# bit-bots/SoccerDiffusion

Hardware: AMD Instinct MI355X
Metric: denoised joint-trajectories/s (50-step DDIM, H=100, J=20) (higher is better)
Workload: dtype f32 (operands split into fp16 hi+lo, 3 fp16 MFMAs per product at every site, fp32 accumulate: 22-bit operands; single noise prediction vs the fp64 oracle 8e-7 on these weights and 2e-6 on weights stressed to |logit| ~ 60 (tests/test_gpu_denoiser.py::test_mode3_noise_prediction_single_step); valid fo; 1 GPU; BASELINE.json configs[2]: 50-step DDIM sampling, B=4096 parallel rollouts per GPU, transformer denoiser d=256 L=4 heads=4, horizon T=100, J=20, memory M=11 (10 context tokens + step token); one step = one full rollout; the timed region issues the rollout's launches eagerly.  Kernel selection: sampler mode 3 (--sampler-mode); batch_per_gpu=4096, ddim_steps=50, horizon=100, joints=20, hidden_dim=256, decoder_layers=4, parallelism=dp1 (independent rollouts, no collective)

## Files before the change

include/soccerdiffusion_hip.h:

```cpp
#ifndef SOCCERDIFFUSION_HIP_H
#define SOCCERDIFFUSION_HIP_H

#include <stddef.h>
#include <stdint.h>

#ifdef __cplusplus
extern "C" {
#endif

#define SD_ABI_VERSION 1

#define SD_E_BADARG (-1)
#define SD_E_BADDIM (-2)
#define SD_E_TOOBIG (-3)
#define SD_E_UNSUPPORTED (-4)

typedef struct sd_layer_weights {
    const float *sa_in_w;
    const float *sa_in_b;
    const float *sa_out_w;
    const float *sa_out_b;
    const float *ca_in_w;
    const float *ca_in_b;
    const float *ca_out_w;
// ... 38 lines not shown
int sd_abi_version(void);
const char *sd_last_error(void);

size_t sd_workspace_floats(int B, int T, int M, int d, int L, int n_steps);

#define SD_ROUTE_CHAINS_F32 0
#define SD_ROUTE_CHAINS_F16 1
#define SD_ROUTE_FUSED 2
#define SD_ROUTE_FUSED_FOLD 3
#define SD_ROUTE_FUSED_FOLD_F16 4
#define SD_ROUTE_TRAJ_TUNED 5
#define SD_ROUTE_TRAJ_TUNED_2P 6
#define SD_ROUTE_TRAJ_TUNED_WIDE 7
#define SD_ROUTE_TRAJ_GENERIC 8
int sd_sampler_route(int d, int heads, int T, int Mc, int J, int L, int B, int max_mode);
int sd_sampler_mode(int d, int heads, int T, int Mc, int J);

int sd_step_token(const void *steps, int steps_is_i64, const float *freq, const float *token,
                  float *out, long out_row_stride, int B, int d, void *stream);

int sd_denoiser_forward(const sd_denoiser_weights *w, const float *x, const float *memory,
                        float *eps_out, float *workspace, int B, int T, int M, void *stream);

int sd_encoder_forward(const sd_encoder_weights *w, const float *x, float *out,
                       float *workspace, int B, int S, void *stream);

int sd_game_state_embed(const int64_t *idx, const float *table, float *out, long out_row_stride,
                        int B, int d, int n_states, void *stream);

int sd_ddim_add_noise(const float *x0, const float *noise, const int64_t *t, const float *acp,
// ... 305 lines not shown
```

soccerdiffusion_amd/_lib.py:

```python

from __future__ import annotations

import ctypes as C
import os

import torch

_PKG = os.path.dirname(os.path.abspath(__file__))
LIB_PATH = os.environ.get("SD_HIP_LIB") or os.path.join(_PKG, "lib", "libsoccerdiffusion_hip.so")

c_float_p = C.POINTER(C.c_float)


class LayerWeights(C.Structure):

    FIELDS = (
        "sa_in_w", "sa_in_b", "sa_out_w", "sa_out_b",
        "ca_in_w", "ca_in_b", "ca_out_w", "ca_out_b",
        "lin1_w", "lin1_b", "lin2_w", "lin2_b",
        "n1_w", "n1_b", "n2_w", "n2_b", "n3_w", "n3_b",
    )
    _fields_ = [(n, C.c_void_p) for n in FIELDS]


# ... 189 lines not shown
    "sd_session_commit_carry_at": (C.c_int, [C.c_void_p] * 7 + [C.c_int] * 7 + [C.c_void_p] * 3),
    "sd_session_reset_carry": (C.c_int, [C.POINTER(RingReset), C.c_int, C.c_void_p, C.c_void_p, C.c_int64, C.c_void_p, C.c_int, C.c_void_p]),
    "sd_profile_enable": (C.c_int, [C.c_int]),
    "sd_profile_collect": (C.c_int, [C.POINTER(C.c_double), C.POINTER(C.c_long), C.c_int]),
}

ROUTES = ("CHAINS_F32", "CHAINS_F16", "FUSED", "FUSED_FOLD", "FUSED_FOLD_F16", "TRAJ_TUNED", "TRAJ_TUNED_2P", "TRAJ_TUNED_WIDE", "TRAJ_GENERIC")


def sampler_route(d: int, heads: int, T: int, Mc: int, J: int, L: int, B: int, max_mode: int = -1) -> str:
    rc = load().sd_sampler_route(d, heads, T, Mc, J, L, B, max_mode)
    check(min(rc, 0), "sd_sampler_route")
    return ROUTES[rc]


KERNEL_CLASSES = ("panel_gemm_kernel", "attention_kernel", "patch_embed_kernel", "fc_out_kernel", "decoder_layer_kernel", "decoder_head_kernel",
                  "traj_step_kernel")

_lib = None


def load() -> C.CDLL:
    global _lib
    if _lib is not None:
        return _lib
    if not os.path.exists(LIB_PATH):
        raise RuntimeError(
            f"{LIB_PATH} is missing: build it with `python -m soccerdiffusion_amd.build` "
            "(hipcc, gfx950).  soccerdiffusion_amd has no CPU fallback."
        )
# ... 17 lines not shown
```

soccerdiffusion_amd/csrc/sd_kernels.hip:

```cpp

#include <hip/hip_runtime.h>
#include <stdint.h>
#include <math.h>
#include <algorithm>
#include <cstdlib>
#include <cstring>

#include "../../include/soccerdiffusion_hip.h"

#include "sd_common.h"
#include "sd_panel.h"

static thread_local const char *g_last_error = "ok";
int fail(int code, const char *msg) {
    g_last_error = msg;
    return code;
}

const unsigned *g_dropout_epoch = nullptr;
extern "C" int sd_set_dropout_epoch(const uint32_t *device_word) {
    g_dropout_epoch = device_word;
    return 0;
}

// ... 2619 lines not shown
        return fail(SD_E_BADDIM, "hidden_dim must be one of 64, 128, 256, 512");
    if (w->p <= 0 || S / w->p <= 0 || S / w->p > w->S_max)
        return fail(SD_E_TOOBIG, "sd_encoder_forward: sequence exceeds positional table");
    hipStream_t st = (hipStream_t)stream;
    const int d = w->d, n = S / w->p, R = B * n;
    Scratch s = carve(workspace, R, 1, d, 1, 0);
    int rc = patch_embed(x, w->emb_w, w->emb_b, w->pe, s.h, B, S, w->C, w->p, d, st);
    if (rc) return rc;
    if ((rc = encoder_stack(w->layers, w->L, s, B, n, d, w->heads, st))) return rc;
    SD_LAUNCH(copy_rows_kernel, dim3(grid_for((long)R * d)), dim3(256), 0, st, s.h, (long)d, out, (long)d,
                       (long)R, d);
    SD_CHECK_LAUNCH("copy_rows_kernel");
    return 0;
}

extern "C" int sd_sampler_mode(int d, int heads, int T, int Mc, int J) { return sampler_plan(d, heads, T, Mc, J, 1, 1, 3).mode(); }

extern "C" int sd_sampler_route(int d, int heads, int T, int Mc, int J, int L, int B, int max_mode) {
    if (max_mode < -1 || max_mode > 4) return fail(SD_E_BADARG, "sd_sampler_route: max_mode must be -1, 0, 1, 2, 3 or 4");
    return sampler_plan(d, heads, T, Mc, J, L, B, max_mode < 0 ? 3 : max_mode).route;
}

extern "C" int sd_ddim_sample(const sd_denoiser_weights *w, const float *ctx, const float *step_tokens,
                              const float *coef, float *x, float *trace, float *workspace, int B, int T, int Mc,
                              int n_steps, void *stream) {
    return sd_ddim_sample_eps(w, ctx, step_tokens, coef, x, trace, nullptr, workspace, B, T, Mc, n_steps, nullptr, -1, stream);
}

extern "C" int sd_ddim_sample_ex(const sd_denoiser_weights *w, const float *ctx, const float *step_tokens,
                                 const float *coef, float *x, float *trace, float *workspace, int B, int T, int Mc,
                                 int n_steps, int32_t *status, int max_mode, void *stream) {
    return sd_ddim_sample_eps(w, ctx, step_tokens, coef, x, trace, nullptr, workspace, B, T, Mc, n_steps, status, max_mode, stream);
}


// ... 38 lines not shown
    const long n = (long)B * T * J;
    SD_LAUNCH(ddim_pin_kernel, dim3(grid_for(n)), dim3(256), 0, st, x, pin, ck, cn, n, T, J);
    SD_CHECK_LAUNCH("ddim_pin_kernel");
    return 0;
}

static int traj_rollout(const TrajCall &c, const float *ctx, const float *step_tokens, const float *coef, float *x, float *trace, float *eps_trace,
                        int32_t *status, const PinArgs *pin = nullptr) {
    const long n = (long)c.B * c.T * c.w->J;
    int rc;
    if (status && (rc = zero_async(status, sizeof(int32_t), c.st))) return rc;
    if ((rc = c.prepare_weights())) return rc;
    if ((rc = c.prepare_ctx(ctx))) return rc;
    if ((rc = c.prepare_steps(step_tokens, false))) return rc;
    if (pin && (rc = ddim_pin(x, *pin, coef[0], coef[1], c.B, c.T, c.w->J, c.st))) return rc;
    for (int i = 0; i < c.n_tok; ++i) {
        float *eps_i = eps_trace ? eps_trace + (size_t)i * n : nullptr;
        if ((rc = c.step(x, eps_i, i, coef + 4 * i, false, status, pin))) return rc;
        if (trace && (rc = trace_copy(x, trace, i, n, c.st))) return rc;
    }
    return status ? finite_check(x, n, status, c.st) : 0;
}

static int panel_rollout(const sd_denoiser_weights *w, const Scratch &s, const SamplerPlan &plan, const float *ctx, const float *step_tokens,
                         const float *coef, float *x, float *trace, float *eps_trace, int B, int T, int Mc, int n_steps, int32_t *status, hipStream_t st,
                         const PinArgs *pin = nullptr) {
    const int d = w->d, R = B * T, L = w->L;
    int rc;
    const int Mk = Mc + 1;
    const size_t kvstride = (size_t)B * Mk * 2 * d, kvsstride = (size_t)n_steps * 2 * d;
// ... 67 lines not shown
}

static int ddim_sample_any(const sd_denoiser_weights *w, const float *ctx, const float *step_tokens, const float *coef, float *x, float *trace,
                           float *eps_trace, float *workspace, int B, int T, int Mc, int n_steps, int32_t *status, int max_mode, void *stream,
                           const PinArgs *pin) {
    int rc = check_denoiser(w);
    if (rc) return rc;
    if (!step_tokens || !coef || !x || !workspace || B <= 0 || T <= 0 || Mc < 0 || n_steps <= 0 || (Mc > 0 && !ctx))
        return fail(SD_E_BADARG, "sd_ddim_sample: null pointer or empty shape");
    if (max_mode < -1 || max_mode > 4) return fail(SD_E_BADARG, "sd_ddim_sample_ex: max_mode must be -1, 0, 1, 2, 3 or 4");
    if (max_mode < 0) max_mode = 3;
    if (max_mode == 4 && !status) return fail(SD_E_BADARG, "sd_ddim_sample_ex: max_mode 4 needs a status word (SD_STATUS_SHARP_LOGITS)");
    if (T > w->T_max) return fail(SD_E_TOOBIG, "sd_ddim_sample: horizon exceeds positional table");
    hipStream_t st = (hipStream_t)stream;
    const Scratch s = carve(workspace, (long)B * T, (long)B * (Mc + 1), w->d, w->L, n_steps, B);
    const SamplerPlan plan = sampler_plan(w->d, w->heads, T, Mc, w->J, w->L, B, max_mode);
    if (plan.traj()) return traj_rollout(TrajCall{plan, w, s, B, T, Mc, n_steps, st}, ctx, step_tokens, coef, x, trace, eps_trace, status, pin);
    return panel_rollout(w, s, plan, ctx, step_tokens, coef, x, trace, eps_trace, B, T, Mc, n_steps, status, st, pin);
}

extern "C" int sd_ddim_sample_eps(const sd_denoiser_weights *w, const float *ctx, const float *step_tokens,
                                  const float *coef, float *x, float *trace, float *eps_trace, float *workspace, int B, int T, int Mc,
                                  int n_steps, int32_t *status, int max_mode, void *stream) {
    return ddim_sample_any(w, ctx, step_tokens, coef, x, trace, eps_trace, workspace, B, T, Mc, n_steps, status, max_mode, stream, nullptr);
}

extern "C" int sd_ddim_sample_pin(const sd_denoiser_weights *w, const float *ctx, const float *step_tokens, const float *coef, float *x,
                                  float *trace, float *eps_trace, float *workspace, int B, int T, int Mc, int n_steps, int32_t *status,
                                  int max_mode, const float *pin_x0, const float *pin_noise, const int32_t *pin_rows, void *stream) {
    if (!pin_x0 || !pin_noise || !pin_rows) return fail(SD_E_BADARG, "sd_ddim_sample_pin: pin_x0, pin_noise and pin_rows must be given");
    if (pin_noise == x) return fail(SD_E_BADARG, "sd_ddim_sample_pin: pin_noise must not alias x (x is overwritten by the first step)");
    const PinArgs pin{pin_x0, pin_noise, pin_rows};
    return ddim_sample_any(w, ctx, step_tokens, coef, x, trace, eps_trace, workspace, B, T, Mc, n_steps, status, max_mode == 4 ? 3 : max_mode,
                           stream, &pin);
}

static int sampler_eval_args(const sd_denoiser_weights *w, float *workspace, int B, int T, int Mc, int n_tok, int max_mode, const char *who,
                             Scratch *s, SamplerPlan *plan) {
    int rc = check_denoiser(w);
    if (rc) return rc;
    if (!workspace || B <= 0 || T <= 0 || Mc < 0 || (n_tok != 1 && n_tok != B)) return fail(SD_E_BADARG, who);
    if (max_mode < -1 || max_mode > 4) return fail(SD_E_BADARG, who);
    if (T > w->T_max) return fail(SD_E_TOOBIG, who);
    *s = carve(workspace, (long)B * T, (long)B * (Mc + 1), w->d, w->L, n_tok, B);
    *plan = sampler_plan(w->d, w->heads, T, Mc, w->J, w->L, B, max_mode < 0 ? 3 : max_mode);
    return plan->traj() ? 0 : SD_E_UNSUPPORTED;
}

extern "C" int sd_sampler_prepare(const sd_denoiser_weights *w, const float *ctx, float *workspace, int B, int T, int Mc, int n_tok,
                                  int what, int max_mode, void *stream) {
    Scratch s;
    SamplerPlan plan;
    int rc = sampler_eval_args(w, workspace, B, T, Mc, n_tok, max_mode, "sd_sampler_prepare: bad argument", &s, &plan);
    if (rc) return rc;
    if ((what & ~(SD_PREPARE_WEIGHTS | SD_PREPARE_CONTEXT)) || (Mc > 0 && (what & SD_PREPARE_CONTEXT) && !ctx))
        return fail(SD_E_BADARG, "sd_sampler_prepare: bad argument");
    const TrajCall c{plan, w, s, B, T, Mc, n_tok, (hipStream_t)stream};
    if ((what & SD_PREPARE_WEIGHTS) && (rc = c.prepare_weights())) return rc;
    if ((what & SD_PREPARE_CONTEXT) && (rc = c.prepare_ctx(ctx))) return rc;
    return 0;
// ... 142 lines not shown
```

soccerdiffusion_amd/csrc/sd_sampler_plan.h:

```cpp
#ifndef SD_SAMPLER_PLAN_H
#define SD_SAMPLER_PLAN_H
#include <stdlib.h>
#include <string.h>

#include "../../include/soccerdiffusion_hip.h"

bool traj_ok(int d, int heads, int T, int Mk, int J, int L);
bool trajg_ok(int d, int heads, int T, int Mk, int J, int L);

inline bool fused_layer_ok(int d, int heads, int T, int Mk) {
    if (heads != 4 || d < 128) return false;
    const int n_traj = (63 + T - 1) / T + 1;
    return (long)n_traj * Mk <= 64;
}

struct SamplerSwitches {
    bool traj, f16, trajg;
    int max_rows;
};
inline const SamplerSwitches &sampler_switches() {
    static const SamplerSwitches sw = [] {
        const auto is = [](const char *name, const char *value) {
            const char *e = getenv(name);
            return e && strcmp(e, value) == 0;
        };
        const char *mr = getenv("SD_TRAJ_MAXROWS");
        return SamplerSwitches{!is("SD_SAMPLER_TRAJ", "0"), !is("SD_SAMPLER_GEMM", "f32"), !is("SD_SAMPLER_TRAJG", "0"), mr ? atoi(mr) : 64};
    }();
    return sw;
}

struct SamplerPlan {
    int route;
    int key_tiles;
    bool precise;
    bool kv_fp32;
    bool fused, fold, f16, chain16;
    bool traj() const { return route >= SD_ROUTE_TRAJ_TUNED; }
    int mode() const { return traj() ? 3 : route == SD_ROUTE_FUSED_FOLD_F16 ? 2 : route == SD_ROUTE_FUSED_FOLD ? 1 : 0; }
};

inline SamplerPlan panel_plan(int d, int heads, int T, int Mk, int J, int B, int cap) {
    const SamplerSwitches &sw = sampler_switches();
    const bool layer_ok = fused_layer_ok(d, heads, T, Mk);
    SamplerPlan p{};
    p.kv_fp32 = cap < 2;
    p.fused = layer_ok && (long)B * Mk * 2 * d < (1L << 30);
    p.fold = cap >= 1 && p.fused && heads == 4 && d >= 128 && Mk <= 16 && T >= 64;
    p.f16 = cap >= 2 && p.fold && sw.f16 && d == 256 && J % 4 == 0;
    p.chain16 = cap >= 2 && !p.fold && !layer_ok && sw.f16 && (d == 128 || d == 256 || d == 512) && J % 4 == 0;
    p.route = p.f16 ? SD_ROUTE_FUSED_FOLD_F16 : p.fold ? SD_ROUTE_FUSED_FOLD : p.fused ? SD_ROUTE_FUSED : p.chain16 ? SD_ROUTE_CHAINS_F16 : SD_ROUTE_CHAINS_F32;
    return p;
}

inline SamplerPlan sampler_plan(int d, int heads, int T, int Mc, int J, int L, int B, int max_mode) {
    const SamplerSwitches &sw = sampler_switches();
    const int Mk = Mc + 1;
    if (max_mode >= 3 && sw.traj && sw.f16) {
        if ((long)B * Mk * 2 * d < (1L << 30) && Mk <= sw.max_rows && traj_ok(d, heads, T, Mk, J, L)) {
            SamplerPlan p{};
            p.key_tiles = (Mk + 15) / 16;
            p.precise = max_mode == 3 || p.key_tiles > 1;
            p.route = p.key_tiles > 1 ? SD_ROUTE_TRAJ_TUNED_WIDE : p.precise ? SD_ROUTE_TRAJ_TUNED : SD_ROUTE_TRAJ_TUNED_2P;
            return p;
        }
        if (sw.trajg && trajg_ok(d, heads, T, Mk, J, L)) {
            SamplerPlan p{};
            p.route = SD_ROUTE_TRAJ_GENERIC;
            return p;
        }
    }
    return panel_plan(d, heads, T, Mk, J, B, max_mode < 2 ? max_mode : 2);
}
#endif
```

soccerdiffusion_amd/csrc/sd_traj.h:

```cpp
#pragma once
#include "sd_common.h"
#include "sd_mfma16.h"
#include "soccerdiffusion_hip.h"
#include <type_traits>

namespace tj {

constexpr int D = 256, HD = 64, NH = 4, TMAX = 100;
constexpr int NTHREADS = 512;
constexpr int MAX_L = 8;
constexpr float ACT = 8.0f;
constexpr float PSC = 1024.0f;
constexpr float XSC = 1.0f;
constexpr int XROW = 1024, X1ROW = 512, QROW = 256, VROW = 288, PROW = 512;
constexpr int LDS_X = 0;
constexpr int LDS_SQ = LDS_X + TMAX * X1ROW;
constexpr int LDS_SO = LDS_SQ + TMAX * QROW;
constexpr int LDS_Q = LDS_X + TMAX * XROW;
constexpr int LDS_K = LDS_Q + TMAX * QROW;
constexpr int LDS_P = LDS_Q;
constexpr int LDS_STAT = LDS_K + TMAX * VROW;
constexpr int LDS_BYTES = LDS_STAT + TMAX * 8 * 8;
static_assert(LDS_SO + TMAX * QROW <= LDS_Q, "Q and O fit the freed half of the panel");
static_assert(LDS_BYTES <= 163840 && LDS_P + TMAX * PROW <= LDS_STAT, "LDS budget");
// ... 6 lines not shown
constexpr int TJ_NSTAMP = 96, TJ_STAMP_WGS = 512;
__device__ unsigned long long *g_tj_stamps;
#define TJ_STAMP(i)                                                                                                            \
    do {                                                                                                                       \
        if (blockIdx.x < TJ_STAMP_WGS && (threadIdx.x & 63) == 0)                                                              \
            g_tj_stamps[((long)blockIdx.x * 8 + (threadIdx.x >> 6)) * TJ_NSTAMP + (i)] = __builtin_amdgcn_s_memtime();        \
    } while (0)
template <int SITE>
__device__ __forceinline__ void tj_sync() {
    const unsigned long long t0 = __builtin_amdgcn_s_memtime();
    __syncthreads();
    const unsigned long long t1 = __builtin_amdgcn_s_memtime();
    if (blockIdx.x < TJ_STAMP_WGS && (threadIdx.x & 63) == 0) g_tj_stamps[((long)blockIdx.x * 8 + (threadIdx.x >> 6)) * TJ_NSTAMP + 64 + SITE] += t1 - t0;
}
#define TJ_SYNC(site) tj_sync<site>()
#else
#define TJ_STAMP(i) do {} while (0)
#define TJ_SYNC(site) __syncthreads()
#endif

#ifndef TJ_DROP_ALO
#define TJ_DROP_ALO 0
#endif
#ifndef TJ_DROP_BLO
#define TJ_DROP_BLO 0
#endif
enum Site { S_QKV = 1, S_SCORES = 2, S_PV = 4, S_OUT = 8, S_XSC = 16, S_XPV = 32, S_W1 = 64, S_W2 = 128, S_EMB = 256, S_FC = 512 };
template <int SITE = 0>
__device__ __forceinline__ void mma3(f32x4 &c, f16x8 ah, f16x8 al, f16x8 bh, f16x8 bl) {
    if constexpr ((TJ_DROP_ALO | TJ_DROP_BLO) & SITE) {
        if constexpr (!(TJ_DROP_ALO & SITE)) c = mfma16(al, bh, c);
        if constexpr (!(TJ_DROP_BLO & SITE)) c = mfma16(ah, bl, c);
        c = mfma16(ah, bh, c);
// ... 171 lines not shown
    const float *b_emb, *pe;
    const float *n1_w, *n1_b;
    const f16 *w_out;
    const float *b_out;
    const float *sc_io;
    float c0, c1, c2, c3;
    float scale_log2e;
    int T, B, J, L, Mk, update_x;
    int nkt;
    const int *step_map;
    int step_per_traj;
    int *status;
    LayerW layer[MAX_L];
};

template <int NTT, bool PRECISE>
struct TJ {
static constexpr int LAST0 = 16 * (NTT - 1);
static constexpr int NH0 = (NTT + 1) / 2;
static constexpr int NKP = (NTT + 1) / 2;


static __device__ __forceinline__ void ctx_init(Ctx &c, char *smem, int T) {
    c.smem = smem;
    c.lane = threadIdx.x & 63;
    c.w = __builtin_amdgcn_readfirstlane(threadIdx.x >> 6);
    c.g = c.lane >> 4;
    c.t = c.lane & 15;
    c.T = T;
    c.ok6 = LAST0 + c.t < T;
    c.tok6 = c.ok6 ? LAST0 + c.t : T - 1;
#pragma unroll
    for (int m2 = 0; m2 < 4; ++m2) {
        const unsigned in_row = (unsigned)(((c.g ^ (c.t & 3)) << 4) + ((m2 ^ (c.t >> 2)) << 6));
        const unsigned in_row6 = (unsigned)(((c.g ^ (c.tok6 & 3)) << 4) + ((m2 ^ ((c.tok6 >> 2) & 3)) << 6));
        c.xa[m2] = (unsigned)(c.t * XROW) + in_row;
        c.xa6[m2] = (unsigned)(c.tok6 * XROW) + in_row6;
    }
}

static __device__ __forceinline__ Ctx ctx_local(const Ctx &c) {
    Ctx d;
    d.smem = c.smem;
    d.lane = c.lane;
    asm volatile("" : "+v"(d.lane));
    d.w = c.w;
    d.g = d.lane >> 4;
    d.t = d.lane & 15;
    d.T = c.T;
    d.ok6 = LAST0 + d.t < d.T;
    d.tok6 = d.ok6 ? LAST0 + d.t : d.T - 1;
#pragma unroll
    for (int m2 = 0; m2 < 4; ++m2) {
// ... 782 lines not shown
            for (int pl = 0; pl < 2; ++pl) svv[n][pl] = vstep[(pl * 4 + c.g) * D + 16 * (2 * c.w + n) + c.t];
        }
        __builtin_amdgcn_sched_barrier(0);
        auto scores = [&](auto odd_c) __attribute__((always_inline)) {
            constexpr bool OD = decltype(odd_c)::value;
            constexpr int N1 = OD ? NTT - NH0 : NH0, T1 = OD ? NH0 : 0;
            constexpr int N1D = N1 > 0 ? N1 : 1;
            f16x8 xb[3][2];
            ring_pipe<8 * N1, 3>(
                [&](int s) __attribute__((always_inline)) {
                    xb[s % 3][0] = lds16(X + x_at(c, T1 + s % N1D, 0, s / N1D));
                    xb[s % 3][1] = lds16(X + x_at(c, T1 + s % N1D, 1, s / N1D));
                },
                [&](int s) __attribute__((always_inline)) { mma3<S_XSC>(S[s % N1D], gfr[s / N1D][0], gfr[s / N1D][1], xb[s % 3][0], xb[s % 3][1]); });
        };
        if (odd) scores(std::true_type{});
        else scores(std::false_type{});
#pragma unroll
        for (int n = 0; n < 2; ++n)
#pragma unroll
            for (int pl = 0; pl < 2; ++pl) av[n][2][pl] = f16x8{svv[n][pl], 0, 0, 0, 0, 0, 0, 0};
        const float c_g = 1.0f / (ACT * sc4);
        const StepScale ss = step_scale(sc5, sc6, sc7);
        f32x4 cg4 = {c_g, c_g, c_g, c_g};
#pragma unroll
        for (int r = 0; r < 4; ++r)
            if (4 * c.g + r == Mc) {
                cbv[r] = cs;
                cg4[r] = ss.c_gs;
            }
// ... 72 lines not shown
            store_x(c, tt, gl[0], gl[1]);
            __builtin_amdgcn_sched_barrier(0);
        }
        TJ_SYNC(7);
        TJ_STAMP(37);
        const float up = ACT * sc2;
        scale_h(H, up);
        gemm_x2<S_W2>(c, H, L.w_2);
        unscale_h(H, 1.0f / up, b2);
    }
    TJ_STAMP(38);
    if (L.nln_w) layer_norm_to_x<!PRECISE>(c0, H, L.nln_w, L.nln_b);
    TJ_STAMP(39);
}

template <bool WIDE = false, bool PIN = false>
static __device__ __forceinline__ void step_body(const StepArgs &a, const PinArgs &pin = PinArgs{}) {
    extern __shared__ __attribute__((aligned(16))) char smem[];
    Ctx c;
    ctx_init(c, smem, a.T);
    const long traj = blockIdx.x;
    const int J = a.J;
    TJ_STAMP(0);
    f32x4 H[2][NTT];
    {
        char *Qb = c.smem + LDS_Q;
        f16x8 we[2][2];
        f32x4 be[2], pe4[2][NTT];
#pragma unroll
        for (int n = 0; n < 2; ++n) {
            const f16 *wp = a.w_emb + (long)(2 * c.w + n) * (2 * 512) + c.lane * 8;
            we[n][0] = *reinterpret_cast<const f16x8 *>(wp);
            we[n][1] = *reinterpret_cast<const f16x8 *>(wp + 512);
            const int n0 = 32 * c.w + 16 * n + 4 * c.g;
            be[n] = *reinterpret_cast<const f32x4 *>(a.b_emb + n0);
#pragma unroll
            for (int tt = 0; tt < NTT; ++tt) pe4[n][tt] = *reinterpret_cast<const f32x4 *>(a.pe + (long)tok_of(c, tt) * D + n0);
        }
        __builtin_amdgcn_sched_barrier(0);
        const float *xr = a.x + traj * (long)a.T * J;
        if (J & 3) {
            for (int i = threadIdx.x; i < a.T * 4; i += NTHREADS) {
                const int tok = i >> 2, chunk = i & 3;
                f16x8 h8, l8;
#pragma unroll
                for (int e = 0; e < 8; ++e) {
                    const int j = 8 * chunk + e;
                    const float v = j < J ? xr[tok * J + j] * XSC : 0.f;
                    h8[e] = (f16)v;
                    l8[e] = (f16)(v - (float)h8[e]);
                }
                *reinterpret_cast<f16x8 *>(Qb + q_off(tok, chunk)) = h8;
                *reinterpret_cast<f16x8 *>(Qb + q_off(tok, chunk | 4)) = l8;
            }
        }
        const int nvec = (J & 3) ? 0 : a.T * J / 4;
        for (int i = threadIdx.x; i < nvec; i += NTHREADS) {
            const f32x4 v = *reinterpret_cast<const f32x4 *>(xr + 4 * i) * XSC;
            const int tok = (4 * i) / J, j0 = 4 * i - tok * J;
            const int chunk = j0 >> 3;
            split_store(Qb + q_off(tok, chunk) + 2 * (j0 & 7), Qb + q_off(tok, chunk | 4) + 2 * (j0 & 7), v);
            if (j0 + 4 >= J) {
                const f16x4 z4 = {0, 0, 0, 0};
                for (int k = J; k < 32; k += 4) {
                    *reinterpret_cast<f16x4 *>(Qb + q_off(tok, k >> 3) + 2 * (k & 7)) = z4;
                    *reinterpret_cast<f16x4 *>(Qb + q_off(tok, (k >> 3) | 4) + 2 * (k & 7)) = z4;
                }
            }
        }
        TJ_SYNC(8);
        const float c_e = 1.0f / (XSC * a.sc_io[0]);
#pragma unroll
        for (int n = 0; n < 2; ++n) {
            const f16x8 ah = we[n][0], al = we[n][1];
#pragma unroll
            for (int tt = 0; tt < NTT; ++tt) {
                f32x4 acc = {0.f, 0.f, 0.f, 0.f};
                mma3<S_EMB>(acc, ah, al, lds16(Qb + q_at(c, tt, 0, 0)), lds16(Qb + q_at(c, tt, 1, 0)));
                H[n][tt] = acc * c_e + (be[n] + pe4[n][tt]);
            }
        }
    }
    TJ_STAMP(1);
    layer_norm_to_x<!PRECISE>(c, H, a.n1_w, a.n1_b);
    TJ_STAMP(2);
#pragma unroll 1
    for (int l = 0; l < a.L; ++l) decoder_layer<WIDE>(c, a.layer[l], H, traj, a.Mk, a.scale_log2e, a.status, a.nkt, a.step_per_traj ? (a.step_map ? (long)a.step_map[traj] : traj) : 0L);
    {
        float *stat = reinterpret_cast<float *>(c.smem + LDS_STAT);
        int pin_rows = 0;
        if constexpr (PIN) pin_rows = pin.rows[traj];
        float am[NTT];
#pragma unroll
        for (int tt = 0; tt < NTT; ++tt) {
            const f32x4 a0 = H[0][tt], a1 = H[1][tt];
            float m = fmaxf(fmaxf(fabsf(a0[0]), fabsf(a0[1])), fmaxf(fabsf(a0[2]), fabsf(a0[3])));
            m = fmaxf(m, fmaxf(fmaxf(fabsf(a1[0]), fabsf(a1[1])), fmaxf(fabsf(a1[2]), fabsf(a1[3]))));
            am[tt] = rows4_max(m);
        }
        if (c.g == 0) {
#pragma unroll
            for (int tt = 0; tt < NTT; ++tt)
                if (tok_ok(c, tt)) stat[tok_of(c, tt) * 8 + c.w] = am[tt];
// ... 3 lines not shown
        for (int tt = 0; tt < NTT; ++tt) {
            const float *sp = stat + tok_of(c, tt) * 8;
            const f32x4 p0 = *reinterpret_cast<const f32x4 *>(sp), p1 = *reinterpret_cast<const f32x4 *>(sp + 4);
            const float m = fmaxf(fmaxf(fmaxf(p0[0], p0[1]), fmaxf(p0[2], p0[3])), fmaxf(fmaxf(p1[0], p1[1]), fmaxf(p1[2], p1[3])));
            const float s = f16_scale_from_bits(__builtin_bit_cast(unsigned, m));
            store_x(c, tt, H[0][tt] * s, H[1][tt] * s);
        }
        f16x8 wf[2][8][2];
        if (c.w < NTT) {
#pragma unroll
            for (int n = 0; n < 2; ++n)
#pragma unroll
                for (int ks = 0; ks < 8; ++ks)
#pragma unroll
                    for (int pl = 0; pl < 2; ++pl) wf[n][ks][pl] = *reinterpret_cast<const f16x8 *>(a.w_out + ((long)(n * 8 + ks) * 2 + pl) * 512 + c.lane * 8);
        }
        __builtin_amdgcn_sched_barrier(0);
        TJ_SYNC(10);
        if (c.w < NTT) {
            const char *X = c.smem + LDS_X;
            f32x4 E[2] = {f32x4{0.f, 0.f, 0.f, 0.f}, f32x4{0.f, 0.f, 0.f, 0.f}};
            const int tok = c.w < NTT - 1 ? 16 * c.w + c.t : c.tok6;
            const bool ok = c.w < NTT - 1 || c.ok6;
#pragma unroll
            for (int ks = 0; ks < 8; ++ks) {
                const int m2lo = (ks & 1) << 1;
                const unsigned b0 = (c.w < NTT - 1 ? c.xa[m2lo] + (unsigned)(c.w * 16 * XROW) : c.xa6[m2lo]) + (unsigned)((ks >> 1) * 256);
                const unsigned b1 = (c.w < NTT - 1 ? c.xa[m2lo | 1] + (unsigned)(c.w * 16 * XROW) : c.xa6[m2lo | 1]) + (unsigned)((ks >> 1) * 256);
                const f16x8 bh = lds16(X + b0), bl = lds16(X + b1);
#pragma unroll
// ... 9 lines not shown
                if (!ok || j0 >= J) continue;
                const long at = (traj * a.T + tok) * J + j0;
                bool pinned = false;
                if constexpr (PIN) pinned = tok < pin_rows;
                if (J & 3) {
#pragma unroll
                    for (int r = 0; r < 4; ++r) {
                        if (j0 + r >= J) continue;
                        const float e = E[n][r] * c_o + a.b_out[j0 + r];
                        if (a.eps_out) a.eps_out[at + r] = e;
                        if constexpr (PIN) {
                            if (a.update_x && pinned) {
                                a.x[at + r] = a.c2 * pin.x0[at + r] + a.c3 * pin.noise[at + r];
                                continue;
                            }
                        }
                        if (a.update_x) {
                            const float x0 = (a.x[at + r] - a.c1 * e) / a.c0;
                            a.x[at + r] = a.c2 * x0 + a.c3 * e;
                        }
                    }
                    continue;
                }
                const f32x4 e = E[n] * c_o + *reinterpret_cast<const f32x4 *>(a.b_out + j0);
                if (a.eps_out) *reinterpret_cast<f32x4 *>(a.eps_out + at) = e;
                if constexpr (PIN) {
                    if (a.update_x && pinned) {
                        const f32x4 k = *reinterpret_cast<const f32x4 *>(pin.x0 + at), nz = *reinterpret_cast<const f32x4 *>(pin.noise + at);
                        *reinterpret_cast<f32x4 *>(a.x + at) = a.c2 * k + a.c3 * nz;
                        continue;
                    }
                }
                if (a.update_x) {
                    const f32x4 xv = *reinterpret_cast<const f32x4 *>(a.x + at);
                    f32x4 xn;
#pragma unroll
                    for (int r = 0; r < 4; ++r) {
                        const float x0 = (xv[r] - a.c1 * e[r]) / a.c0;
                        xn[r] = a.c2 * x0 + a.c3 * e[r];
                    }
                    *reinterpret_cast<f32x4 *>(a.x + at) = xn;
                }
            }
        }
    }
    TJ_STAMP(40);
}
};

template <int NTT, bool PRECISE>
__global__ __launch_bounds__(NTHREADS, 2) void traj_step_kernel(StepArgs a) { TJ<NTT, PRECISE>::step_body(a); }
template <int NTT>
__global__ __launch_bounds__(NTHREADS, 2) void traj_step_wide_kernel(StepArgs a) { TJ<NTT, true>::template step_body<true>(a); }
template <int NTT>
__global__ __launch_bounds__(NTHREADS, 2) void traj_step_pin_kernel(StepArgs a, PinArgs pin) { TJ<NTT, true>::template step_body<false, true>(a, pin); }
template <int NTT>
__global__ __launch_bounds__(NTHREADS, 2) void traj_step_wide_pin_kernel(StepArgs a, PinArgs pin) { TJ<NTT, true>::template step_body<true, true>(a, pin); }


}
```

soccerdiffusion_amd/csrc/sd_traj.hip:

```cpp

#include <hip/hip_runtime.h>
#include <math.h>

#include "../../include/soccerdiffusion_hip.h"

#include "sd_common.h"
#include "sd_traj.h"
#include "sd_traj_host.h"

bool traj_ok(int d, int heads, int T, int Mk, int J, int L) {
    return d == 256 && heads == 4 && T >= 1 && T <= tj::TMAX && Mk >= 1 && Mk <= 64 && J >= 1 && J <= 32 && L >= 1 && L <= tj::MAX_L;
}

typedef void (*TrajStepFn)(tj::StepArgs);
static TrajStepFn traj_step_wide_fn(int ntt) {
    switch (ntt) {
        case 1: return tj::traj_step_wide_kernel<1>;
        case 2: return tj::traj_step_wide_kernel<2>;
        case 3: return tj::traj_step_wide_kernel<3>;
        case 4: return tj::traj_step_wide_kernel<4>;
        case 5: return tj::traj_step_wide_kernel<5>;
        case 6: return tj::traj_step_wide_kernel<6>;
        case 7: return tj::traj_step_wide_kernel<7>;
        default: return nullptr;
    }
}
template <bool PRECISE>
static TrajStepFn traj_step_fn(int ntt) {
    switch (ntt) {
        case 1: return tj::traj_step_kernel<1, PRECISE>;
        case 2: return tj::traj_step_kernel<2, PRECISE>;
        case 3: return tj::traj_step_kernel<3, PRECISE>;
        case 4: return tj::traj_step_kernel<4, PRECISE>;
        case 5: return tj::traj_step_kernel<5, PRECISE>;
        case 6: return tj::traj_step_kernel<6, PRECISE>;
        case 7: return tj::traj_step_kernel<7, PRECISE>;
        default: return nullptr;
    }
}

typedef void (*TrajStepPinFn)(tj::StepArgs, PinArgs);
static TrajStepPinFn traj_step_pin_fn(int ntt, bool wide) {
    switch (ntt) {
        case 1: return wide ? tj::traj_step_wide_pin_kernel<1> : tj::traj_step_pin_kernel<1>;
        case 2: return wide ? tj::traj_step_wide_pin_kernel<2> : tj::traj_step_pin_kernel<2>;
        case 3: return wide ? tj::traj_step_wide_pin_kernel<3> : tj::traj_step_pin_kernel<3>;
        case 4: return wide ? tj::traj_step_wide_pin_kernel<4> : tj::traj_step_pin_kernel<4>;
        case 5: return wide ? tj::traj_step_wide_pin_kernel<5> : tj::traj_step_pin_kernel<5>;
        case 6: return wide ? tj::traj_step_wide_pin_kernel<6> : tj::traj_step_pin_kernel<6>;
        case 7: return wide ? tj::traj_step_wide_pin_kernel<7> : tj::traj_step_pin_kernel<7>;
        default: return nullptr;
// ... 201 lines not shown
        fa.wkv[l] = lw.ca_in_w + (size_t)d * d; fa.bkv[l] = lw.ca_in_b + d;
        fa.wq[l] = lw.ca_in_w; fa.bq[l] = lw.ca_in_b; fa.woc[l] = lw.ca_out_w;
    }
    SD_LAUNCH(step_kv_kernel, dim3((unsigned)n_tok, (unsigned)L, 8), dim3(256), 0, st, fa, tokens, s.kvstep, (long)n_tok, map);
    SD_CHECK_LAUNCH("step_kv_kernel");
    SD_LAUNCH(step_fold_all_kernel, dim3((unsigned)n_tok, (unsigned)L, 4), dim3(256), 0, st, fa, s.kvstep, (long)n_tok, s.gvstep, (long)gvsstride, s.cstep,
              (long)cssstride, s.maxbits, map);
    SD_CHECK_LAUNCH("step_fold_all_kernel");
    unsigned gx = grid_for((long)n_tok * 4 * (d / 8 + d));
    SD_LAUNCH(pack_step16_all_kernel, dim3(gx, (unsigned)L), dim3(256), 0, st, s.gvstep, (long)gvsstride, (long)n_tok, s.maxbits, s.gstep16,
              (long)((size_t)n_tok * 4 * blk), s.vstep16, (long)((size_t)n_tok * blk), s.scales, Mc == 0 ? 1 : 0, map);
    SD_CHECK_LAUNCH("pack_step16_all_kernel");
    return 0;
}

int traj_step(const sd_denoiser_weights *w, const TrajWs &s, float *x, float *eps, int B, int T, int Mc, int i, int n_steps, const float *coef,
              bool per_traj, hipStream_t st, int nkt, bool precise, int32_t *status, const PinArgs *pin) {
    const int d = w->d, L = w->L;
    const size_t blk = (size_t)32 * d, cbstride = (size_t)B * nkt * 64;
    tj::StepArgs a{};
    a.nkt = nkt;
    a.status = status;
    a.x = x;
    a.eps_out = eps;
    a.w_emb = s.wio;
    a.b_emb = w->emb_b;
    a.pe = w->pe;
    a.n1_w = w->layers[0].n1_w;
    a.n1_b = w->layers[0].n1_b;
    a.w_out = s.wio + (size_t)2 * 32 * d;
    a.b_out = w->out_b;
    a.sc_io = s.scales + L * 8 + 6;
// ... 6 lines not shown
        const sd_layer_weights &lw = w->layers[l];
        tj::LayerW &q = a.layer[l];
        q.n2_w = lw.n2_w; q.n2_b = lw.n2_b; q.n3_w = lw.n3_w; q.n3_b = lw.n3_b;
        q.w_o = f16_wf(s.wf, l, d, 0); q.w_1 = f16_wf(s.wf, l, d, 1); q.w_2 = f16_wf(s.wf, l, d, 2); q.w_in = f16_wf(s.wf, l, d, 3);
        q.b_in = lw.sa_in_b; q.b_o = lw.sa_out_b; q.b_1 = lw.lin1_b; q.b_2 = lw.lin2_b; q.b_oc = lw.ca_out_b;
        q.sc = s.scales + l * 8;
        q.g16 = s.g16 + (size_t)l * B * nkt * 4 * blk;
        q.v16 = s.v16 + (size_t)l * B * nkt * 4 * blk;
        q.cb = s.cb + l * cbstride;
        q.gstep = s.gstep16 + (size_t)l * n_steps * 4 * blk + (size_t)i * (4 * 8 * 2 * 32);
        q.vstep = s.vstep16 + (size_t)l * n_steps * blk + (size_t)i * (2 * 4 * d);
        q.cstep = s.cstep + ((size_t)l * n_steps + i) * 4;
        q.nln_w = l + 1 < L ? w->layers[l + 1].n1_w : nullptr;
        q.nln_b = l + 1 < L ? w->layers[l + 1].n1_b : nullptr;
    }
    const int ntt = (T + 15) / 16;
    const int variant = nkt > 1 ? 2 : (precise ? 1 : 0);
    const TrajStepFn fn = variant == 2 ? traj_step_wide_fn(ntt) : (precise ? traj_step_fn<true>(ntt) : traj_step_fn<false>(ntt));
    if (!fn) return fail(SD_E_BADARG, "traj_step_kernel: horizon out of range");
    if (pin) {
        if (!coef || variant == 0) return fail(SD_E_BADARG, "traj_step_pin_kernel: pinned rows need the DDIM coefficients and the three-product kernels");
        const TrajStepPinFn pfn = traj_step_pin_fn(ntt, variant == 2);
        ProfScope prof(SD_KCLASS_TRAJ_STEP, st);
        static DevFlag pin_attr_set[2][8];
        if (!pin_attr_set[variant - 1][ntt]) {
            const hipError_t e = hipFuncSetAttribute((const void *)pfn, hipFuncAttributeMaxDynamicSharedMemorySize, tj::LDS_BYTES);
            if (e != hipSuccess) return fail((int)e, "traj_step_pin_kernel: hipFuncSetAttribute(MaxDynamicSharedMemorySize)");
            pin_attr_set[variant - 1][ntt] = true;
        }
        SD_LAUNCH(pfn, dim3((unsigned)B), dim3(tj::NTHREADS), (size_t)tj::LDS_BYTES, st, a, *pin);
        SD_CHECK_LAUNCH("traj_step_pin_kernel");
        return 0;
    }
    ProfScope prof(SD_KCLASS_TRAJ_STEP, st);
    static DevFlag attr_set[3][8];
    if (!attr_set[variant][ntt]) {
        const hipError_t e = hipFuncSetAttribute((const void *)fn, hipFuncAttributeMaxDynamicSharedMemorySize, tj::LDS_BYTES);
        if (e != hipSuccess) return fail((int)e, "traj_step_kernel: hipFuncSetAttribute(MaxDynamicSharedMemorySize)");
        attr_set[variant][ntt] = true;
    }
    SD_LAUNCH(fn, dim3((unsigned)B), dim3(tj::NTHREADS), (size_t)tj::LDS_BYTES, st, a);
    SD_CHECK_LAUNCH("traj_step_kernel");
    return 0;
}
```

soccerdiffusion_amd/csrc/sd_traj_host.h:

```cpp
#ifndef SD_TRAJ_HOST_H
#define SD_TRAJ_HOST_H
#include "sd_common.h"
#include "sd_sampler_plan.h"
struct sd_denoiser_weights;

struct TrajWs {
    float *kvtmp, *kvstep;
    float *gv, *cb, *gvstep, *cstep;
    f16 *wf, *g16, *v16, *gstep16, *vstep16, *wio;
    float *scales;
    unsigned *maxbits;
    int *stepmap;
};

int traj_prepare_weights(const sd_denoiser_weights *w, const TrajWs &s, hipStream_t st);
int traj_prepare_ctx(const sd_denoiser_weights *w, const TrajWs &s, const float *ctx, int B, int Mc, int nkt, hipStream_t st);
int traj_prepare_steps(const sd_denoiser_weights *w, const TrajWs &s, const float *tokens, int n_tok, int Mc, hipStream_t st, bool per_traj = false);
int traj_step(const sd_denoiser_weights *w, const TrajWs &s, float *x, float *eps, int B, int T, int Mc, int i, int n_tok, const float *coef,
              bool per_traj, hipStream_t st, int nkt, bool precise, int32_t *status, const PinArgs *pin = nullptr);
#endif
```

Measured before the change: 15490 trajectories/s.

## Fuse all DDIM steps of a rollout into one persistent trajectory kernel

Adds a rollout kernel that loops over every DDIM step inside one launch per trajectory block, with the per-step coefficients passed in the kernel arguments. The sampler now takes this path by default when there is no trace, pin or per-step output. It removes the per-step kernel launches and the re-entry into each step, and it preloads x for the DDIM update. The cost is a larger kernel argument block, a block-wide sync between steps, and context rebuilt inside the loop, which could affect register pressure.

```diff
diff --git a/include/soccerdiffusion_hip.h b/include/soccerdiffusion_hip.h
--- a/include/soccerdiffusion_hip.h
+++ b/include/soccerdiffusion_hip.h
@@ -76,6 +76,12 @@
 #define SD_ROUTE_TRAJ_TUNED_WIDE 7
 #define SD_ROUTE_TRAJ_GENERIC 8
 int sd_sampler_route(int d, int heads, int T, int Mc, int J, int L, int B, int max_mode);
+#define SD_ASK_ROLLOUT 0x100
+#define SD_ASK_TRACE 0x10
+#define SD_ASK_PIN 0x20
+#define SD_ASK_LOOP 0x40
+#define SD_ROLLOUT_PER_STEP 0
+#define SD_ROLLOUT_FUSED 1
 int sd_sampler_mode(int d, int heads, int T, int Mc, int J);
 
 int sd_step_token(const void *steps, int steps_is_i64, const float *freq, const float *token,
diff --git a/soccerdiffusion_amd/_lib.py b/soccerdiffusion_amd/_lib.py
--- a/soccerdiffusion_amd/_lib.py
+++ b/soccerdiffusion_amd/_lib.py
@@ -227,6 +227,17 @@
     return ROUTES[rc]
 
 
+ROLLOUTS = ("PER_STEP", "FUSED")
+
+
+def sampler_rollout(d: int, heads: int, T: int, Mc: int, J: int, L: int, B: int, max_mode: int = -1, *, trace: bool = False, pin: bool = False,
+                    loop: bool = False) -> str:
+    ask = 0x100 + (3 if max_mode < 0 else max_mode) + (0x10 if trace else 0) + (0x20 if pin else 0) + (0x40 if loop else 0)
+    rc = load().sd_sampler_route(d, heads, T, Mc, J, L, B, ask)
+    check(min(rc, 0), "sd_sampler_route")
+    return ROLLOUTS[rc]
+
+
 KERNEL_CLASSES = ("panel_gemm_kernel", "attention_kernel", "patch_embed_kernel", "fc_out_kernel", "decoder_layer_kernel", "decoder_head_kernel",
                   "traj_step_kernel")
 
diff --git a/soccerdiffusion_amd/csrc/sd_kernels.hip b/soccerdiffusion_amd/csrc/sd_kernels.hip
--- a/soccerdiffusion_amd/csrc/sd_kernels.hip
+++ b/soccerdiffusion_amd/csrc/sd_kernels.hip
@@ -2657,11 +2657,18 @@
     return 0;
 }
 
-extern "C" int sd_sampler_mode(int d, int heads, int T, int Mc, int J) { return sampler_plan(d, heads, T, Mc, J, 1, 1, 3).mode(); }
+extern "C" int sd_sampler_mode(int d, int heads, int T, int Mc, int J) { return sampler_plan(d, heads, T, Mc, J, 1, 1, 3, CALL_ROLLOUT).mode(); }
 
 extern "C" int sd_sampler_route(int d, int heads, int T, int Mc, int J, int L, int B, int max_mode) {
+    int call = -1;
+    if (max_mode >= SD_ASK_ROLLOUT && max_mode < 2 * SD_ASK_ROLLOUT) {
+        call = (max_mode & SD_ASK_TRACE ? CALL_TRACE : 0) | (max_mode & SD_ASK_PIN ? CALL_PIN : 0) | (max_mode & SD_ASK_LOOP ? CALL_LOOP : 0);
+        max_mode &= 7;
+        if ((call & CALL_PIN) && max_mode == 4) max_mode = 3;
+    }
     if (max_mode < -1 || max_mode > 4) return fail(SD_E_BADARG, "sd_sampler_route: max_mode must be -1, 0, 1, 2, 3 or 4");
-    return sampler_plan(d, heads, T, Mc, J, L, B, max_mode < 0 ? 3 : max_mode).route;
+    const SamplerPlan plan = sampler_plan(d, heads, T, Mc, J, L, B, max_mode < 0 ? 3 : max_mode, call < 0 ? CALL_ROLLOUT : call);
+    return call < 0 ? plan.route : plan.rollout_fused ? SD_ROLLOUT_FUSED : SD_ROLLOUT_PER_STEP;
 }
 
 extern "C" int sd_ddim_sample(const sd_denoiser_weights *w, const float *ctx, const float *step_tokens,
@@ -2730,6 +2737,14 @@
     if ((rc = c.prepare_ctx(ctx))) return rc;
     if ((rc = c.prepare_steps(step_tokens, false))) return rc;
     if (pin && (rc = ddim_pin(x, *pin, coef[0], coef[1], c.B, c.T, c.w->J, c.st))) return rc;
+    if (c.plan.rollout_fused) {
+        if (trace || eps_trace || pin || c.generic()) return fail(SD_E_BADARG, "traj_rollout: the plan's rollout kernel returns nothing per step and has no pin");
+        for (int i0 = 0; i0 < c.n_tok; i0 += TRAJ_ROLLOUT_MAX_STEPS) {
+            const int nn = c.n_tok - i0 < TRAJ_ROLLOUT_MAX_STEPS ? c.n_tok - i0 : TRAJ_ROLLOUT_MAX_STEPS;
+            if ((rc = traj_steps_fused(c.w, c.ws(), x, c.B, c.T, c.Mc, i0, nn, c.n_tok, coef, c.st, c.plan.precise, c.plan.precise ? nullptr : status))) return rc;
+        }
+        return status ? finite_check(x, n, status, c.st) : 0;
+    }
     for (int i = 0; i < c.n_tok; ++i) {
         float *eps_i = eps_trace ? eps_trace + (size_t)i * n : nullptr;
         if ((rc = c.step(x, eps_i, i, coef + 4 * i, false, status, pin))) return rc;
@@ -2827,7 +2842,8 @@
     if (T > w->T_max) return fail(SD_E_TOOBIG, "sd_ddim_sample: horizon exceeds positional table");
     hipStream_t st = (hipStream_t)stream;
     const Scratch s = carve(workspace, (long)B * T, (long)B * (Mc + 1), w->d, w->L, n_steps, B);
-    const SamplerPlan plan = sampler_plan(w->d, w->heads, T, Mc, w->J, w->L, B, max_mode);
+    const int call = ((trace || eps_trace) ? CALL_TRACE : 0) | (pin ? CALL_PIN : 0);
+    const SamplerPlan plan = sampler_plan(w->d, w->heads, T, Mc, w->J, w->L, B, max_mode, call);
     if (plan.traj()) return traj_rollout(TrajCall{plan, w, s, B, T, Mc, n_steps, st}, ctx, step_tokens, coef, x, trace, eps_trace, status, pin);
     return panel_rollout(w, s, plan, ctx, step_tokens, coef, x, trace, eps_trace, B, T, Mc, n_steps, status, st, pin);
 }
@@ -2856,7 +2872,7 @@
     if (max_mode < -1 || max_mode > 4) return fail(SD_E_BADARG, who);
     if (T > w->T_max) return fail(SD_E_TOOBIG, who);
     *s = carve(workspace, (long)B * T, (long)B * (Mc + 1), w->d, w->L, n_tok, B);
-    *plan = sampler_plan(w->d, w->heads, T, Mc, w->J, w->L, B, max_mode < 0 ? 3 : max_mode);
+    *plan = sampler_plan(w->d, w->heads, T, Mc, w->J, w->L, B, max_mode < 0 ? 3 : max_mode, CALL_LOOP);
     return plan->traj() ? 0 : SD_E_UNSUPPORTED;
 }
 
diff --git a/soccerdiffusion_amd/csrc/sd_sampler_plan.h b/soccerdiffusion_amd/csrc/sd_sampler_plan.h
--- a/soccerdiffusion_amd/csrc/sd_sampler_plan.h
+++ b/soccerdiffusion_amd/csrc/sd_sampler_plan.h
@@ -17,6 +17,7 @@
 struct SamplerSwitches {
     bool traj, f16, trajg;
     int max_rows;
+    bool rollout;
 };
 inline const SamplerSwitches &sampler_switches() {
     static const SamplerSwitches sw = [] {
@@ -25,13 +26,22 @@
             return e && strcmp(e, value) == 0;
         };
         const char *mr = getenv("SD_TRAJ_MAXROWS");
-        return SamplerSwitches{!is("SD_SAMPLER_TRAJ", "0"), !is("SD_SAMPLER_GEMM", "f32"), !is("SD_SAMPLER_TRAJG", "0"), mr ? atoi(mr) : 64};
+        return SamplerSwitches{!is("SD_SAMPLER_TRAJ", "0"), !is("SD_SAMPLER_GEMM", "f32"), !is("SD_SAMPLER_TRAJG", "0"), mr ? atoi(mr) : 64,
+                               !is("SD_TRAJ_ROLLOUT", "steps")};
     }();
     return sw;
 }
 
+enum SamplerCall {
+    CALL_ROLLOUT = 0,
+    CALL_TRACE = 1,
+    CALL_PIN = 2,
+    CALL_LOOP = 4,
+};
+
 struct SamplerPlan {
     int route;
+    bool rollout_fused;
     int key_tiles;
     bool precise;
     bool kv_fp32;
@@ -53,7 +63,7 @@
     return p;
 }
 
-inline SamplerPlan sampler_plan(int d, int heads, int T, int Mc, int J, int L, int B, int max_mode) {
+inline SamplerPlan sampler_plan(int d, int heads, int T, int Mc, int J, int L, int B, int max_mode, int call) {
     const SamplerSwitches &sw = sampler_switches();
     const int Mk = Mc + 1;
     if (max_mode >= 3 && sw.traj && sw.f16) {
@@ -62,6 +72,7 @@
             p.key_tiles = (Mk + 15) / 16;
             p.precise = max_mode == 3 || p.key_tiles > 1;
             p.route = p.key_tiles > 1 ? SD_ROUTE_TRAJ_TUNED_WIDE : p.precise ? SD_ROUTE_TRAJ_TUNED : SD_ROUTE_TRAJ_TUNED_2P;
+            p.rollout_fused = sw.rollout && p.key_tiles == 1 && call == CALL_ROLLOUT;
             return p;
         }
         if (sw.trajg && trajg_ok(d, heads, T, Mk, J, L)) {
diff --git a/soccerdiffusion_amd/csrc/sd_traj.h b/soccerdiffusion_amd/csrc/sd_traj.h
--- a/soccerdiffusion_amd/csrc/sd_traj.h
+++ b/soccerdiffusion_amd/csrc/sd_traj.h
@@ -44,9 +44,11 @@
     if (blockIdx.x < TJ_STAMP_WGS && (threadIdx.x & 63) == 0) g_tj_stamps[((long)blockIdx.x * 8 + (threadIdx.x >> 6)) * TJ_NSTAMP + 64 + SITE] += t1 - t0;
 }
 #define TJ_SYNC(site) tj_sync<site>()
+#define TJ_WAIT_FIRST_KEY() asm volatile("s_waitcnt vmcnt(28)" ::: "memory")
 #else
 #define TJ_STAMP(i) do {} while (0)
 #define TJ_SYNC(site) __syncthreads()
+#define TJ_WAIT_FIRST_KEY() do {} while (0)
 #endif
 
 #ifndef TJ_DROP_ALO
@@ -248,6 +250,16 @@
     LayerW layer[MAX_L];
 };
 
+constexpr int ROLL_MAX_STEPS = 64;
+struct RollArgs {
+    int n_steps;
+    float coef[ROLL_MAX_STEPS][4];
+};
+struct RolloutArgs {
+    StepArgs a;
+    RollArgs r;
+};
+
 template <int NTT, bool PRECISE>
 struct TJ {
 static constexpr int LAST0 = 16 * (NTT - 1);
@@ -271,6 +283,15 @@
         c.xa[m2] = (unsigned)(c.t * XROW) + in_row;
         c.xa6[m2] = (unsigned)(c.tok6 * XROW) + in_row6;
     }
+}
+
+static __device__ __forceinline__ Ctx ctx_fresh(char *smem, int wave, int T) {
+    Ctx c1;
+    c1.smem = smem;
+    asm volatile("v_mbcnt_lo_u32_b32 %0, -1, 0\n\tv_mbcnt_hi_u32_b32 %0, -1, %0" : "=v"(c1.lane));
+    c1.w = wave;
+    c1.T = T;
+    return ctx_local(c1);
 }
 
 static __device__ __forceinline__ Ctx ctx_local(const Ctx &c) {
@@ -1083,6 +1104,8 @@
                 },
                 [&](int s) __attribute__((always_inline)) { mma3<S_XSC>(S[s % N1D], gfr[s / N1D][0], gfr[s / N1D][1], xb[s % 3][0], xb[s % 3][1]); });
         };
+        TJ_WAIT_FIRST_KEY();
+        TJ_STAMP(53);
         if (odd) scores(std::true_type{});
         else scores(std::false_type{});
 #pragma unroll
@@ -1185,11 +1208,19 @@
     TJ_STAMP(39);
 }
 
-template <bool WIDE = false, bool PIN = false>
-static __device__ __forceinline__ void step_body(const StepArgs &a, const PinArgs &pin = PinArgs{}) {
+static __device__ __forceinline__ float ddim_update(float x, float e, const f32x4 &k) {
+    const float x0 = __builtin_fmaf(-k[1], e, x) / k[0];
+    const float ce = k[3] * e;
+    return __builtin_fmaf(k[2], x0, ce);
+}
+
+template <bool WIDE = false, bool PIN = false, bool ROLL = false>
+static __device__ __forceinline__ void step_body(const StepArgs &a, const PinArgs &pin = PinArgs{}, f32x4 roll_coef = f32x4{0.f, 0.f, 0.f, 0.f},
+                                                 int roll_step = 0, int roll_wave = 0) {
     extern __shared__ __attribute__((aligned(16))) char smem[];
     Ctx c;
-    ctx_init(c, smem, a.T);
+    if constexpr (ROLL) c = ctx_fresh(smem, roll_wave, a.T);
+    else ctx_init(c, smem, a.T);
     const long traj = blockIdx.x;
     const int J = a.J;
     TJ_STAMP(0);
@@ -1210,8 +1241,9 @@
         }
         __builtin_amdgcn_sched_barrier(0);
         const float *xr = a.x + traj * (long)a.T * J;
+        const int tid = ROLL ? 64 * c.w + c.lane : (int)threadIdx.x;
         if (J & 3) {
-            for (int i = threadIdx.x; i < a.T * 4; i += NTHREADS) {
+            for (int i = tid; i < a.T * 4; i += NTHREADS) {
                 const int tok = i >> 2, chunk = i & 3;
                 f16x8 h8, l8;
 #pragma unroll
@@ -1226,7 +1258,7 @@
             }
         }
         const int nvec = (J & 3) ? 0 : a.T * J / 4;
-        for (int i = threadIdx.x; i < nvec; i += NTHREADS) {
+        for (int i = tid; i < nvec; i += NTHREADS) {
             const f32x4 v = *reinterpret_cast<const f32x4 *>(xr + 4 * i) * XSC;
             const int tok = (4 * i) / J, j0 = 4 * i - tok * J;
             const int chunk = j0 >> 3;
@@ -1256,8 +1288,13 @@
     layer_norm_to_x<!PRECISE>(c, H, a.n1_w, a.n1_b);
     TJ_STAMP(2);
 #pragma unroll 1
-    for (int l = 0; l < a.L; ++l) decoder_layer<WIDE>(c, a.layer[l], H, traj, a.Mk, a.scale_log2e, a.status, a.nkt, a.step_per_traj ? (a.step_map ? (long)a.step_map[traj] : traj) : 0L);
+    for (int l = 0; l < a.L; ++l) decoder_layer<WIDE>(c, a.layer[l], H, traj, a.Mk, a.scale_log2e, a.status, a.nkt,
+                                                           ROLL ? (long)roll_step : a.step_per_traj ? (a.step_map ? (long)a.step_map[traj] : traj) : 0L);
+    const Ctx &c_step = c;
     {
+        Ctx c_tail;
+        if constexpr (ROLL) c_tail = ctx_fresh(smem, roll_wave, a.T);
+        const Ctx &c = ROLL ? c_tail : c_step;
         float *stat = reinterpret_cast<float *>(c.smem + LDS_STAT);
         int pin_rows = 0;
         if constexpr (PIN) pin_rows = pin.rows[traj];
@@ -1291,6 +1328,15 @@
                 for (int ks = 0; ks < 8; ++ks)
 #pragma unroll
                     for (int pl = 0; pl < 2; ++pl) wf[n][ks][pl] = *reinterpret_cast<const f16x8 *>(a.w_out + ((long)(n * 8 + ks) * 2 + pl) * 512 + c.lane * 8);
+        }
+        f32x4 xpre[2] = {f32x4{0.f, 0.f, 0.f, 0.f}, f32x4{0.f, 0.f, 0.f, 0.f}};
+        if constexpr (ROLL) {
+            if (c.w < NTT && !(J & 3) && (c.w < NTT - 1 || c.ok6)) {
+                const int tok = c.w < NTT - 1 ? 16 * c.w + c.t : c.tok6;
+#pragma unroll
+                for (int n = 0; n < 2; ++n)
+                    if (16 * n + 4 * c.g < J) xpre[n] = *reinterpret_cast<const f32x4 *>(a.x + (traj * a.T + tok) * J + 16 * n + 4 * c.g);
+            }
         }
         __builtin_amdgcn_sched_barrier(0);
         TJ_SYNC(10);
@@ -1330,6 +1376,10 @@
                                 a.x[at + r] = a.c2 * pin.x0[at + r] + a.c3 * pin.noise[at + r];
                                 continue;
                             }
+                        }
+                        if constexpr (ROLL) {
+                            if (a.update_x) a.x[at + r] = ddim_update(a.x[at + r], e, roll_coef);
+                            continue;
                         }
                         if (a.update_x) {
                             const float x0 = (a.x[at + r] - a.c1 * e) / a.c0;
@@ -1348,12 +1398,16 @@
                     }
                 }
                 if (a.update_x) {
-                    const f32x4 xv = *reinterpret_cast<const f32x4 *>(a.x + at);
+                    const f32x4 xv = ROLL ? xpre[n] : *reinterpret_cast<const f32x4 *>(a.x + at);
                     f32x4 xn;
 #pragma unroll
                     for (int r = 0; r < 4; ++r) {
-                        const float x0 = (xv[r] - a.c1 * e[r]) / a.c0;
-                        xn[r] = a.c2 * x0 + a.c3 * e[r];
+                        if constexpr (ROLL) {
+                            xn[r] = ddim_update(xv[r], e[r], roll_coef);
+                        } else {
+                            const float x0 = (xv[r] - a.c1 * e[r]) / a.c0;
+                            xn[r] = a.c2 * x0 + a.c3 * e[r];
+                        }
                     }
                     *reinterpret_cast<f32x4 *>(a.x + at) = xn;
                 }
@@ -1361,6 +1415,7 @@
         }
     }
     TJ_STAMP(40);
+    if constexpr (ROLL) __syncthreads();
 }
 };
 
@@ -1372,6 +1427,19 @@
 __global__ __launch_bounds__(NTHREADS, 2) void traj_step_pin_kernel(StepArgs a, PinArgs pin) { TJ<NTT, true>::template step_body<false, true>(a, pin); }
 template <int NTT>
 __global__ __launch_bounds__(NTHREADS, 2) void traj_step_wide_pin_kernel(StepArgs a, PinArgs pin) { TJ<NTT, true>::template step_body<true, true>(a, pin); }
-
-
-}
+template <int NTT, bool PRECISE>
+__global__ __launch_bounds__(NTHREADS, 2) void traj_step_rollout_kernel(RolloutArgs) {
+    typedef const __attribute__((address_space(4))) RolloutArgs *KernArg;
+    const int wave = __builtin_amdgcn_readfirstlane(threadIdx.x >> 6);
+    const int n_steps = ((KernArg)__builtin_amdgcn_kernarg_segment_ptr())->r.n_steps;
+#pragma unroll 1
+    for (int i = 0; i < n_steps; ++i) {
+        KernArg ka = (KernArg)__builtin_amdgcn_kernarg_segment_ptr();
+        asm volatile("" : "+s"(ka));
+        const RolloutArgs &k = *(const RolloutArgs *)ka;
+        TJ<NTT, PRECISE>::template step_body<false, false, true>(k.a, PinArgs{}, f32x4{k.r.coef[i][0], k.r.coef[i][1], k.r.coef[i][2], k.r.coef[i][3]}, i, wave);
+    }
+}
+
+
+}
diff --git a/soccerdiffusion_amd/csrc/sd_traj.hip b/soccerdiffusion_amd/csrc/sd_traj.hip
--- a/soccerdiffusion_amd/csrc/sd_traj.hip
+++ b/soccerdiffusion_amd/csrc/sd_traj.hip
@@ -35,6 +35,21 @@
         case 5: return tj::traj_step_kernel<5, PRECISE>;
         case 6: return tj::traj_step_kernel<6, PRECISE>;
         case 7: return tj::traj_step_kernel<7, PRECISE>;
+        default: return nullptr;
+    }
+}
+
+typedef void (*TrajRolloutFn)(tj::RolloutArgs);
+template <bool PRECISE>
+static TrajRolloutFn traj_rollout_fn(int ntt) {
+    switch (ntt) {
+        case 1: return tj::traj_step_rollout_kernel<1, PRECISE>;
+        case 2: return tj::traj_step_rollout_kernel<2, PRECISE>;
+        case 3: return tj::traj_step_rollout_kernel<3, PRECISE>;
+        case 4: return tj::traj_step_rollout_kernel<4, PRECISE>;
+        case 5: return tj::traj_step_rollout_kernel<5, PRECISE>;
+        case 6: return tj::traj_step_rollout_kernel<6, PRECISE>;
+        case 7: return tj::traj_step_rollout_kernel<7, PRECISE>;
         default: return nullptr;
     }
 }
@@ -266,8 +281,8 @@
     return 0;
 }
 
-int traj_step(const sd_denoiser_weights *w, const TrajWs &s, float *x, float *eps, int B, int T, int Mc, int i, int n_steps, const float *coef,
-              bool per_traj, hipStream_t st, int nkt, bool precise, int32_t *status, const PinArgs *pin) {
+static tj::StepArgs step_args(const sd_denoiser_weights *w, const TrajWs &s, float *x, float *eps, int B, int T, int Mc, int i, int n_steps, const float *coef,
+                              bool per_traj, int nkt, int32_t *status) {
     const int d = w->d, L = w->L;
     const size_t blk = (size_t)32 * d, cbstride = (size_t)B * nkt * 64;
     tj::StepArgs a{};
@@ -304,6 +319,12 @@
         q.nln_w = l + 1 < L ? w->layers[l + 1].n1_w : nullptr;
         q.nln_b = l + 1 < L ? w->layers[l + 1].n1_b : nullptr;
     }
+    return a;
+}
+
+int traj_step(const sd_denoiser_weights *w, const TrajWs &s, float *x, float *eps, int B, int T, int Mc, int i, int n_steps, const float *coef,
+              bool per_traj, hipStream_t st, int nkt, bool precise, int32_t *status, const PinArgs *pin) {
+    const tj::StepArgs a = step_args(w, s, x, eps, B, T, Mc, i, n_steps, coef, per_traj, nkt, status);
     const int ntt = (T + 15) / 16;
     const int variant = nkt > 1 ? 2 : (precise ? 1 : 0);
     const TrajStepFn fn = variant == 2 ? traj_step_wide_fn(ntt) : (precise ? traj_step_fn<true>(ntt) : traj_step_fn<false>(ntt));
@@ -333,3 +354,29 @@
     SD_CHECK_LAUNCH("traj_step_kernel");
     return 0;
 }
+
+int traj_steps_fused(const sd_denoiser_weights *w, const TrajWs &s, float *x, int B, int T, int Mc, int i0, int n, int n_steps, const float *coef,
+                     hipStream_t st, bool precise, int32_t *status) {
+    static_assert(TRAJ_ROLLOUT_MAX_STEPS == tj::ROLL_MAX_STEPS, "one cap on both sides of the interface");
+    static_assert(sizeof(tj::RolloutArgs) <= 4096, "kernel argument");
+    if (n < 1 || n > tj::ROLL_MAX_STEPS || i0 < 0 || i0 + n > n_steps || !coef) return fail(SD_E_BADARG, "traj_step_rollout_kernel: bad step range");
+    tj::RolloutArgs ra{};
+    ra.a = step_args(w, s, x, nullptr, B, T, Mc, i0, n_steps, coef + 4 * i0, false, 1, status);
+    tj::RollArgs &r = ra.r;
+    r.n_steps = n;
+    for (int i = 0; i < n; ++i)
+        for (int k = 0; k < 4; ++k) r.coef[i][k] = coef[4 * (i0 + i) + k];
+    const int ntt = (T + 15) / 16;
+    const TrajRolloutFn fn = precise ? traj_rollout_fn<true>(ntt) : traj_rollout_fn<false>(ntt);
+    if (!fn) return fail(SD_E_BADARG, "traj_step_rollout_kernel: horizon out of range");
+    ProfScope prof(SD_KCLASS_TRAJ_STEP, st);
+    static DevFlag attr_set[2][8];
+    if (!attr_set[precise ? 1 : 0][ntt]) {
+        const hipError_t e = hipFuncSetAttribute((const void *)fn, hipFuncAttributeMaxDynamicSharedMemorySize, tj::LDS_BYTES);
+        if (e != hipSuccess) return fail((int)e, "traj_step_rollout_kernel: hipFuncSetAttribute(MaxDynamicSharedMemorySize)");
+        attr_set[precise ? 1 : 0][ntt] = true;
+    }
+    SD_LAUNCH(fn, dim3((unsigned)B), dim3(tj::NTHREADS), (size_t)tj::LDS_BYTES, st, ra);
+    SD_CHECK_LAUNCH("traj_step_rollout_kernel");
+    return 0;
+}
diff --git a/soccerdiffusion_amd/csrc/sd_traj_host.h b/soccerdiffusion_amd/csrc/sd_traj_host.h
--- a/soccerdiffusion_amd/csrc/sd_traj_host.h
+++ b/soccerdiffusion_amd/csrc/sd_traj_host.h
@@ -18,4 +18,7 @@
 int traj_prepare_steps(const sd_denoiser_weights *w, const TrajWs &s, const float *tokens, int n_tok, int Mc, hipStream_t st, bool per_traj = false);
 int traj_step(const sd_denoiser_weights *w, const TrajWs &s, float *x, float *eps, int B, int T, int Mc, int i, int n_tok, const float *coef,
               bool per_traj, hipStream_t st, int nkt, bool precise, int32_t *status, const PinArgs *pin = nullptr);
+constexpr int TRAJ_ROLLOUT_MAX_STEPS = 64;
+int traj_steps_fused(const sd_denoiser_weights *w, const TrajWs &s, float *x, int B, int T, int Mc, int i0, int n, int n_tok, const float *coef,
+                     hipStream_t st, bool precise, int32_t *status);
 #endif
```

Measured after the change: 15990 trajectories/s, median of 6. 3.2% higher.
